# itsakeyfut/renderer-rs

Measured on AMD Instinct MI355X. Metric: Mtris/s at 1920x1080 (input triangles per second, whole frame incl. shading + store), higher is better.
Workload: dtype f32+i32; 1 GPU; c2: BASELINE configs[1]: 10k random triangles, flat shade, 1920x1080; triangles=10000, width=1920, height=1080, target_format=B8G8R8A8_SRGB, parallelism=single, frames_in_flight=4, queue_lanes=4

## Files before the change

renderer-rs_amd/csrc/mirhi_api.hip:

```cpp
#include <hip/hip_runtime.h>

#include <algorithm>
#include <atomic>
#include <chrono>
#include <condition_variable>
#include <cmath>
#include <cstdarg>
#include <cstdio>
#include <cstdlib>
#include <cstring>
#include <mutex>
#include <new>
#include <string>
#include <thread>
#include <vector>

#include <dlfcn.h>
#include <hsa/hsa.h>
#include <hsa/hsa_ext_amd.h>
#include <hsa/amd_hsa_signal.h>
#include <rccl/rccl.h>

#include "../../include/mirhi.h"
#include "mirhi_device.h"
// ... 2108 lines not shown
            j.vb = dd.vb; j.camera = dd.camera; j.object = dd.object; j.stride = dd.stride; j.count = count;
            j.words = words; j.slot_base = slots;
            slots += (count + GEOM_THREADS - 1) / GEOM_THREADS * GEOM_THREADS;
            v.jobs.push_back(j); v.out_off.push_back(v.out_bytes);
            v.out_bytes += vs_attr_offset(count) + (((size_t)count * (words - 1u) * 16 + 255) & ~(size_t)255);
            found = v.jobs.size() - 1;
        }
        dd.vs_words = v.jobs[found].words;
        dd.vs_out = (const void*)(uintptr_t)(v.out_off[found] + 1);
        dd.vs_attr = (const void*)(uintptr_t)(v.out_off[found] + vs_attr_offset(v.jobs[found].count) + 1);
    }
    return v;
}

static mirhi_result grow_scope_buffers(Workspace& w, const std::vector<RecordedPass>& passes, const std::vector<ScopePlan>& scopes, const std::vector<VertexPlan>& vertex) {
    mirhi_result r;
    size_t vs_bytes = 0, carry = 0, ord = 0, flat_tris = 0, pd = 0;
    for (size_t pi = 0; pi < passes.size(); pi++) {
        const RecordedPass& pass = passes[pi];
        vs_bytes = std::max(vs_bytes, vertex[pi].out_bytes);
        if ((pass.carry_in || pass.carry_out) && !pass.depth_t.ptr) carry = std::max(carry, (size_t)pass.color_t.width * pass.color_t.height * 4);
        if (scopes[pi].cls.ordered) ord = std::max(ord, scopes[pi].tris * sizeof(TriRec));
        if (scopes[pi].cls.tri_prog && pass.color_t.format == MIRHI_FORMAT_B8G8R8A8_SRGB) flat_tris = std::max<size_t>(flat_tris, pass.total_tris);
        if (pass.draws.size() > 1) pd = std::max(pd, scopes[pi].tris);
    }
    if ((r = grow(&w.vs_out, &w.vs_out_bytes, vs_bytes ? vs_bytes : 256)) != MIRHI_OK) return r;
    if (carry && (r = grow(&w.carry_depth, &w.carry_depth_bytes, carry)) != MIRHI_OK) return r;
    if (ord && (r = grow(&w.ordered, &w.ordered_bytes, ord)) != MIRHI_OK) return r;
    if (flat_tris && (r = grow(&w.flat_color, &w.flat_color_bytes, flat_tris * 4)) != MIRHI_OK) return r;
    if (pd && (r = grow(&w.prim_draw, &w.prim_draw_bytes, pd * 4)) != MIRHI_OK) return r;
    return MIRHI_OK;
}

static PassParams fill_params(const RecordedPass& pass, const ScopePlan& s, const RasterMode& mode, const Workspace& w, size_t max_tiles, unsigned long long* frag_stats) {
    const RecordedPass::Target& ci = pass.color_t;
    const size_t pool_pages = w.bin_pool_bytes / (BIN_PAGE_RECS * sizeof(BinRec));
    PassParams P;
    memset(&P, 0, sizeof P);
    P.width = ci.width; P.height = ci.height;
    P.tiles_x = s.tiles_x; P.tiles_y = s.tiles_y; P.tile_row_begin = s.r0; P.tile_row_end = s.r1; P.tile_row_step = s.rstep;
    P.num_draws = (uint32_t)pass.draws.size(); P.total_tris = pass.total_tris;
    set_raster_choice(P, s.cls, mode, pass.state, w.ordered, pass.first_tri, pass.total_tris);
    memcpy(P.clear_color, pass.info.clear_color, sizeof P.clear_color);
    {
        auto sat = [](float c) { return c > 0.0f ? (c < 1.0f ? c : 1.0f) : 0.0f; };
        auto enc = [&](float c) { c = sat(c); float e = c <= 0.0031308f ? 12.92f * c : 1.055f * std::pow(c, 1.0f / 2.4f) - 0.055f; return (uint32_t)std::nearbyint(sat(e) * 255.0f); };
        P.clear_packed = enc(P.clear_color[2]) | (enc(P.clear_color[1]) << 8) | (enc(P.clear_color[0]) << 16) |
                         ((uint32_t)std::nearbyint(sat(P.clear_color[3]) * 255.0f) << 24);
    }
    P.color_load = pass.info.color_load_op == MIRHI_LOAD_OP_LOAD ? 1u : 0u;
    P.color_format = ci.format;
    P.color = const_cast<uint8_t*>(ci.ptr);
    if (pass.depth_t.ptr) {
        P.depth = (float*)const_cast<uint8_t*>(pass.depth_t.ptr);
        P.depth_load = pass.info.depth_load_op == MIRHI_LOAD_OP_LOAD ? 1u : 0u;
        P.depth_store = pass.info.depth_store_op == MIRHI_STORE_OP_STORE ? 1u : 0u;
    } else if (pass.carry_in || pass.carry_out) {
        P.depth = w.carry_depth;
    }
    if (pass.carry_in) P.depth_load = 1u;
    if (pass.carry_out) P.depth_store = 1u;
    P.prim_out = (uint32_t*)const_cast<uint8_t*>(pass.prim_t.ptr);
    P.bin_pool = w.bin_pool; P.bin_count = w.counters + CTR_BINS; P.bin_cap = s.bins.bin_cap;
    P.bin_table = w.bin_table; P.pool_next = w.counters + CTR_POOL;
    P.pool_dyn_base = s.bins.fixed_pages; P.pool_dyn_pages = (uint32_t)((pool_pages - s.bins.fixed_pages) / 8);
    P.fixed_recs = s.bins.fixed_per_tile * BIN_PAGE_RECS;
    P.big_recs = w.big_recs; P.big_count = w.big_counts; P.big_count_next = w.big_counts + 1; P.big_cap = s.bins.big_cap;
    P.status = w.status_dev;
    P.frag_stats = frag_stats;
    P.first_prim = pass.first_tri;
    P.prim_draw = pass.draws.size() > 1 ? w.prim_draw : nullptr;
    P.flat_color = (s.cls.tri_prog && ci.format == MIRHI_FORMAT_B8G8R8A8_SRGB) ? w.flat_color : nullptr;
    P.resolve_flat_only = (P.flat_color && !P.depth_load && P.color_format != 2u && !P.prim_out && !(P.depth && P.depth_store)) ? 1u : 0u;
    P.sub_cap = s.bins.sub_cap;
    P.count_stride = s.mode.xcd_bins ? (uint32_t)max_tiles : 0u;
    P.depth_only = pass.depth_only ? 1u : 0u;
    if (P.ibl) {
        P.ibl_irradiance = (const float*)pass.ibl.irradiance; P.ibl_prefiltered = (const float*)pass.ibl.prefiltered; P.ibl_lut = (const float*)pass.ibl.lut;
        P.ibl_irr_size = pass.ibl.irr_size; P.ibl_pre_size = pass.ibl.pre_size; P.ibl_pre_levels = pass.ibl.pre_levels; P.ibl_lut_size = pass.ibl.lut_size;
    }
    if (P.sky) {
        const RecordedPass::SkyDraw& k = pass.sky;
        P.sky_visible = k.visible; P.sky_size = k.size; P.sky_levels = k.levels; P.sky_env = (const float*)k.env;
        memcpy(P.sky_a, k.a, sizeof P.sky_a); memcpy(P.sky_b, k.b, sizeof P.sky_b); memcpy(P.sky_scissor, k.scissor, sizeof P.sky_scissor);
        for (int i = 0; i < 3; i++) P.sky_e0[i] = k.e0[i];
        memcpy(P.sky_pos0, k.pos0, sizeof P.sky_pos0); memcpy(P.sky_posx, k.posx, sizeof P.sky_posx); memcpy(P.sky_posy, k.posy, sizeof P.sky_posy);
        P.sky_depth_bits = k.depth_bits; P.sky_compare = k.compare; P.sky_write = k.write; P.sky_prim = k.prim;
    }
    return P;
}

static mirhi_result build_plan(mirhi_cmd* cmd, bool in_submit) {
    const PlanKnobs knobs = PlanKnobs::read();
    mirhi_device* dev = cmd->dev;
    HIP_TRY(hipSetDevice(dev->ordinal));
    if (cmd->lane >= dev->lanes.size()) cmd->lane = 0;
    hipStream_t stream = dev->lanes[cmd->lane];
    cmd->plan_valid = false;
    { mirhi_result rs = settle_pending(cmd, in_submit); if (rs != MIRHI_OK) return rs; }
    Workspace& w = cmd->ws;
    const size_t n = cmd->passes.size();
    {
        uint64_t tris_now = 0;
        for (auto& pass : cmd->passes) tris_now += pass.total_tris - pass.first_tri;
        if (w.spread && (tris_now > 2 * w.spread_tris || 2 * tris_now < w.spread_tris)) w.spread = false;
    }
    mirhi_result r;
    std::vector<ScopePlan> scopes;
    size_t total_draws = 0, max_tiles = 0;
    for (const RecordedPass& pass : cmd->passes) {
        scopes.push_back(plan_scope(dev, pass, w, knobs));
        total_draws += pass.draws.size();
        max_tiles = std::max(max_tiles, scopes.back().tiles());
    }
    if ((r = rearm_workspace(cmd, scopes, max_tiles, stream, knobs)) != MIRHI_OK) return r;
    std::vector<VertexPlan> vertex;
    size_t jobs_total = 0;
    for (const RecordedPass& pass : cmd->passes) { vertex.push_back(vertex_jobs(pass)); jobs_total += vertex.back().jobs.size(); }
    if ((r = grow_scope_buffers(w, cmd->passes, scopes, vertex)) != MIRHI_OK) return r;
    const size_t params_bytes = n * 2 * sizeof(PassParams);
    w.draws_off = (params_bytes + 255) & ~(size_t)255;
    w.jobs_off = (w.draws_off + total_draws * sizeof(DrawDesc) + 255) & ~(size_t)255;
    const size_t block_bytes = w.jobs_off + jobs_total * sizeof(VsJob);
    if ((r = pblock_reserve(w, block_bytes ? block_bytes : 256)) != MIRHI_OK) return r;
    w.params = reinterpret_cast<PassParams*>(w.pblock);
    DrawDesc* const dev_draws = reinterpret_cast<DrawDesc*>(w.pblock + w.draws_off);
    VsJob* const dev_jobs = reinterpret_cast<VsJob*>(w.pblock + w.jobs_off);
    w.pimage.assign(block_bytes, 0);
    w.draws_count = total_draws;

    size_t draws_done = 0, jobs_done = 0;
    w.wide_eligible = false;
    cmd->plan.clear(); cmd->plan_programs.clear(); cmd->plan_tris = 0;
    for (size_t pi = 0; pi < n; pi++) {
        const ScopePlan& s = scopes[pi];
        VertexPlan& v = vertex[pi];
        const RasterMode mode = raster_mode(s.cls, s.tiles(), s.tris, w.spread, w.wide, knobs);
        w.wide_eligible |= mode.wide_eligible;
        PassParams P = fill_params(cmd->passes[pi], s, mode, w, max_tiles, dev->frag_stats);
        P.draws = dev_draws + draws_done;
        P.vs_jobs = dev_jobs + jobs_done;
        P.num_vs_jobs = (uint32_t)v.jobs.size();
        VsJob* const img_jobs = reinterpret_cast<VsJob*>(w.pimage.data() + w.jobs_off) + jobs_done;
        for (size_t j = 0; j < v.jobs.size(); j++) {
            v.jobs[j].out = w.vs_out + v.out_off[j];
            P.vs_total_slots = v.jobs[j].slot_base + (v.jobs[j].count + GEOM_THREADS - 1) / GEOM_THREADS * GEOM_THREADS;
            img_jobs[j] = v.jobs[j];
        }
        jobs_done += v.jobs.size();
        uint32_t slots = 0;
        for (DrawDesc& dd : v.draws) {
            if (dd.vs_words) { dd.vs_out = w.vs_out + ((size_t)(uintptr_t)dd.vs_out - 1); dd.vs_attr = w.vs_out + ((size_t)(uintptr_t)dd.vs_attr - 1); }
            dd.slot_base = slots; slots += (dd.tri_count + GEOM_THREADS - 1) / GEOM_THREADS * GEOM_THREADS;
        }
        P.total_slots = slots;
        if (!v.draws.empty()) memcpy(w.pimage.data() + w.draws_off + draws_done * sizeof(DrawDesc), v.draws.data(), v.draws.size() * sizeof(DrawDesc));
        draws_done += v.draws.size();
        cmd->plan.push_back(P);
        cmd->plan_programs.push_back(s.cls.programs);
        cmd->plan_tris += s.tris;
        for (uint32_t parity = 0; parity < 2; parity++) {
            PassParams Q = P;
            Q.big_count = w.big_counts + parity;
            Q.big_count_next = w.big_counts + (parity ^ 1u);
            Q.active = w.counters + CTR_ACTIVE + parity * 8u * 32u;
            Q.active_prev = w.counters + CTR_ACTIVE + (parity ^ 1u) * 8u * 32u;
            memcpy(w.pimage.data() + (2 * pi + parity) * sizeof(PassParams), &Q, sizeof Q);
        }
    }
    if ((r = pblock_commit(w, stream)) != MIRHI_OK) return r;
    if (!w.pblock_direct) { cmd->last_stream = stream; cmd->last_native = nullptr; cmd->pending = true; }
    { std::lock_guard<std::mutex> lk(dev->mu); cmd->planned = cmd->passes; }
// ... 1 lines not shown
    cmd->plan_valid = true;
    dev->stats.workspace_bytes = w.bytes();
    return MIRHI_OK;
}

extern "C" int mirhi_debug_raster_choice(const uint32_t in[12], char* name, uint32_t name_len, uint32_t grid_block[4]);
extern "C" int mirhi_debug_scope_plan(const uint32_t* in, uint32_t* out, char* name, uint32_t name_len) {
    static float some_map; static TriRec some_recs;
    const PlanKnobs knobs = PlanKnobs::read();
    DepthState s;
    s.key_set = in[0] != 0u; s.test = in[1]; s.compare = in[2]; s.write = in[3]; s.discard = in[4]; s.blend[0] = in[5];
    float clear_depth; memcpy(&clear_depth, &in[6], 4);
    const uint32_t n = in[14];
    if (n > 4u) return -1;
    DrawDesc draws[4];
    memset(draws, 0, sizeof draws);
    for (uint32_t i = 0; i < n; i++) {
        draws[i].program = in[15 + 3 * i];
        if (in[16 + 3 * i]) { draws[i].shadow_map = &some_map; draws[i].shadow_layers = in[16 + 3 * i] == 2u ? 4u : 0u; }
        draws[i].tex_any_mips = in[17 + 3 * i];
    }
    const ScopeClass c = classify_scope(s, clear_depth, draws, n, in[7] != 0u, knobs, n == 1u && draws[0].program == (uint32_t)MIRHI_PROGRAM_SKYBOX);
    const RasterMode m = raster_mode(c, in[8], in[9], in[10] != 0u, in[11], knobs);
    const BinGeometry g = bin_geometry(in[8], in[9], in[9], m.xcd_bins, in[12], knobs);
    const uint32_t words[28] = {c.key.clear_depth_bits, c.key.pred, c.key.zflip, c.key.zmask, c.key.idflip, c.key.strict, c.key.init_zk, c.key.init_idk,
                                c.ordered, c.masked_plain, c.tri_prog, c.shadowed, c.ibl, c.own_family, c.programs,
                                m.tp_max_area, m.teams, m.wide_eligible, m.xcd_bins, m.wide, m.xcd_swizzle,
                                g.bin_cap, g.sub_cap, g.fixed_per_tile, g.fixed_pages, (uint32_t)g.pages, (uint32_t)((uint64_t)g.pages >> 32), g.big_cap};
    memcpy(out, words, sizeof words);
    PassParams P{};
    set_raster_choice(P, c, m, s, &some_recs, 0u, in[9]);
    const uint32_t choice[12] = {c.programs, in[13], P.pred, P.zflip, P.zmask, P.tp_max_area, P.raster_teams, P.raster_wide, P.alpha_scope, P.xcd_swizzle, P.ordered_recs ? 1u : 0u, 0u};
    return mirhi_debug_raster_choice(choice, name, name_len, out + 28);
}

static mirhi_result stats_params_for(mirhi_cmd* c) {
    Workspace& w = c->ws;
    if (w.stats_params_valid) return MIRHI_OK;
    size_t pixels = 0;
    for (const PassParams& P : c->plan) pixels = std::max(pixels, (size_t)P.width * P.height);
    mirhi_result r;
    if ((r = grow(&w.stats_prim, &w.stats_prim_bytes, (pixels ? pixels : 1) * 4)) != MIRHI_OK) return r;
    if ((r = grow(&w.stats_params, &w.stats_params_bytes, (c->plan.size() ? c->plan.size() : 1) * 2 * sizeof(PassParams))) != MIRHI_OK) return r;
    std::vector<PassParams> copies;
    for (const PassParams& P0 : c->plan)
        for (uint32_t parity = 0; parity < 2; parity++) {
            PassParams P = P0;
            P.big_count = w.big_counts + parity;
            P.big_count_next = w.big_counts + (parity ^ 1u);
            P.active = w.counters + CTR_ACTIVE + parity * 8u * 32u;
            P.active_prev = w.counters + CTR_ACTIVE + (parity ^ 1u) * 8u * 32u;
            P.prim_out = w.stats_prim;
            P.resolve_flat_only = 0u;
            copies.push_back(P);
        }
    if (!copies.empty()) {
        c->dev->foreign_writes++;
        HIP_TRY(hipMemcpyAsync(w.stats_params, copies.data(), copies.size() * sizeof(PassParams), hipMemcpyHostToDevice, c->dev->stream));
        HIP_TRY(hipStreamSynchronize(c->dev->stream));
    }
    w.stats_params_valid = true;
    return MIRHI_OK;
}

static mirhi_result timing_begin(mirhi_device* dev, uint32_t kernel, uint32_t lane, LaunchTiming* t) {
    hipEvent_t ev[2];
// ... 819 lines not shown
```

renderer-rs_amd/csrc/mirhi_device.h:

```cpp
#pragma once
#include <stddef.h>
#include <stdint.h>

namespace mirhi {

constexpr int TILE = 32;
constexpr int TILE_LOG2 = 5;
constexpr int BLOCK = 8;
constexpr int RASTER_THREADS = 256;
constexpr int RASTER_CHUNK = 192;
constexpr int TP_MIN_LANES = 32;
constexpr int GEOM_THREADS = 64;
constexpr int MAX_BIN_SPAN = 4;
constexpr float GUARD_PX = 16000.0f;
constexpr int BIN_PAGE_RECS = 64;
constexpr int BIN_PAGE_LOG2 = 6;
constexpr int BIN_TABLE_ROW = 64;
constexpr int POOL_COUNTER_STRIDE = 32;
constexpr uint32_t BIN_COUNT_STRIDE = 16;
constexpr uint32_t PAGE_EMPTY = 0xFFFFFFFFu;
constexpr uint32_t PAGE_NONE = 0xFFFFFFFEu;
constexpr uint32_t NO_PRIM = 0xFFFFFFFFu;
constexpr uint32_t MAX_PRIM_ID = 0xFFFFFFFDu;

// ... 70 lines not shown
    uint32_t num_draws, total_tris;
    uint32_t total_slots;
    const DrawDesc* draws;
    const VsJob* vs_jobs; uint32_t num_vs_jobs, vs_total_slots;
    uint32_t zflip, zmask, idflip;
    uint32_t strict;
    uint32_t pred;
    uint32_t init_zk, init_idk;
    uint32_t clear_depth_bits;
    float    clear_color[4];
    uint32_t clear_packed;
    uint32_t color_load;
    uint32_t color_format;
    void*    color;
    float*   depth;
    uint32_t depth_load, depth_store;
    uint32_t* prim_out;
    BinRec*   bin_pool; uint32_t* bin_count; uint32_t bin_cap;
    uint32_t* bin_table;
    uint32_t* pool_next;
    uint32_t  pool_dyn_base, pool_dyn_pages;
    uint32_t  fixed_recs;
    BigRec*   big_recs; uint32_t* big_count; uint32_t big_cap;
    uint32_t* big_count_next;
    uint32_t* prim_draw;
    uint32_t  first_prim;
    uint32_t* flat_color;
    uint32_t tp_max_area;
    uint32_t xcd_swizzle;
    uint32_t raster_teams;
    uint32_t sub_cap, count_stride;
    uint32_t raster_wide;
    uint32_t resolve_flat_only;
    uint32_t* active; uint32_t* active_prev;
    TriRec*  ordered_recs; uint32_t ordered_first, ordered_count;
    uint32_t ord_depth_test, ord_depth_write, ord_depth_op;
    uint32_t blend[8];
    uint32_t alpha_scope;
    uint32_t* status;
    unsigned long long* frag_stats;
    uint32_t depth_only;
    uint32_t shadowed;
    uint32_t ibl;
    uint32_t ibl_irr_size, ibl_pre_size, ibl_pre_levels, ibl_lut_size, ibl_pad;
    const float* ibl_irradiance; const float* ibl_prefiltered; const float* ibl_lut;
    uint32_t sky;
    uint32_t sky_visible;
    uint32_t sky_size, sky_levels;
    const float* sky_env;
    int32_t  sky_a[3], sky_b[3];
    int32_t  sky_scissor[4];
    long long sky_e0[3];
    float    sky_pos0[3], sky_posx[3], sky_posy[3];
    uint32_t sky_depth_bits;
    uint32_t sky_compare, sky_write;
    uint32_t sky_prim;
};
static_assert(sizeof(PassParams) % 8 == 0, "PassParams holds pointers");

struct GeometryHead {
    const DrawDesc* draws; uint32_t num_draws;
    uint32_t tris_per_wave;
    const uint8_t* vb0; uint32_t stride0, first0, tris0;
};
struct RasterHead {
    uint32_t* bin_count; const BinRec* bin_pool; uint32_t* big_count;
// ... 12 lines not shown
```

renderer-rs_amd/csrc/mirhi_raster.hip.h:

```cpp
#ifndef MIRHI_RASTER_HIP_H
#define MIRHI_RASTER_HIP_H

#pragma clang fp contract(off)

#ifndef MIRHI_STAGE_PRIO
#define MIRHI_STAGE_PRIO 0
#endif

struct PixelState { uint32_t zk[4], idk[4]; };
struct RecRegs { uint4 w0, w1, w2, w3; };

__device__ __forceinline__ RecRegs load_rec(const uint4* lds_rec, uint32_t j) {
    RecRegs r;
    r.w0 = lds_rec[j * 4u + 0]; r.w1 = lds_rec[j * 4u + 1]; r.w2 = lds_rec[j * 4u + 2]; r.w3 = lds_rec[j * 4u + 3];
    return r;
}

__device__ __forceinline__ int32_t mad24(int32_t a, int32_t b, int32_t c) {
    int32_t d;
    asm("v_mad_i32_i24 %0, %1, %2, %3" : "=v"(d) : "v"(a), "v"(b), "v"(c));
    return d;
}

__device__ __forceinline__ int64_t mul24x24(int32_t a, int32_t b) {
    const uint32_t lo = (uint32_t)__mul24(a, b);
    const int32_t hi = __mulhi(a, b);
    return (int64_t)(((uint64_t)(uint32_t)hi << 32) | lo);
}

struct TileTri { int32_t X[3], Y[3]; uint32_t box, z0, zx, zy, idk, boxed; };
__device__ __forceinline__ uint32_t clamp_box(int32_t bx0, int32_t bx1, int32_t by0, int32_t by1) {
    bx0 = bx0 < 0 ? 0 : (bx0 > TILE ? TILE : bx0); by0 = by0 < 0 ? 0 : (by0 > TILE ? TILE : by0);
    bx1 = bx1 > TILE - 1 ? TILE - 1 : (bx1 < -1 ? -1 : bx1); by1 = by1 > TILE - 1 ? TILE - 1 : (by1 < -1 ? -1 : by1);
    return (uint32_t)bx0 | (((uint32_t)bx1 & 0xFFu) << 8) | ((uint32_t)by0 << 16) | ((uint32_t)by1 << 24);
}

__device__ __forceinline__ bool tile_rec_core(uint4 out[4], const int32_t X[3], const int32_t Y[3], int32_t Ptx, int32_t Pty,
                                              int32_t bx0, int32_t bx1, int32_t by0, int32_t by1, float fox, float foy,
                                              uint32_t z0, uint32_t zx, uint32_t zy, uint32_t idk, uint32_t boxed) {
// ... 321 lines not shown
#pragma unroll 1
        for (int32_t ix = bx0; ix <= bx1; ix++) {
            if ((s0 | s1 | s2) >= 0) {
                const float alpha = pbr_base_alpha(D, c, uvk, px_base + (float)ix, py_base + (float)iy);
                if (!(alpha < cutoff)) {
                    const float dx = (float)ix + dxt;
                    const float z = __builtin_fmaf(dy, zy, __builtin_fmaf(dx, zx, z0));
                    uint32_t zk = __float_as_uint(__builtin_amdgcn_fmed3f(z, 0.0f, 1.0f)) & 0x7FFFFFFFu;
                    if (KEYED == 1) zk = (zk ^ P.zflip) & P.zmask;
                    atomicMin(&lds_key[iy * TILE + ix], ((unsigned long long)zk << 32) | idk);
                }
            }
            s0 += A0; s1 += A1; s2 += A2;
        }
        r0 += B0; r1 += B1; r2 += B2;
    }
}

__device__ __forceinline__ void init_key(ParamsRef P, uint32_t px, uint32_t py, bool valid, uint32_t& zk,
                                         uint32_t& idk, uint32_t& zorig) {
    zk = P.init_zk; idk = P.init_idk; zorig = P.clear_depth_bits;
    if (P.depth_load && P.depth && valid) {
        const uint32_t bits = __float_as_uint(P.depth[(size_t)py * P.width + px]);
        zorig = bits;
        if (P.zmask) {
            const uint32_t t = bits ^ P.zflip;
            if (!P.strict) { zk = t; idk = NO_PRIM; }
            else if (t == 0u) { zk = 0u; idk = 0u; }
            else { zk = t - 1u; idk = NO_PRIM; }
        }
    }
}

template <int KEYED, int TP, int CHUNK, int TEAMS, bool BINS, bool MASKED = false, int WPT = 4>
__device__ __forceinline__ void raster_list(const uint4* __restrict__ list, uint32_t n_total, uint32_t tile, uint32_t fixed_recs, const uint32_t* pages, const uint32_t* seg, uint4* lds_rec, uint32_t* lds_box,
                                            uint32_t* lds_count, uint32_t& flip, uint32_t team, uint32_t nteams, unsigned long long* lds_key, uint32_t tx, uint32_t ty,
                                            uint32_t qmask, int32_t ix0, int32_t iy0, float fix0, float fiy0,
                                            ParamsRef P, PixelState& st, uint32_t qbit0, uint32_t tid,
                                            uint32_t lane) {
    const uint32_t fq = (uint32_t)__builtin_amdgcn_readfirstlane((int)(((tid >> 6) + ((tx + ty) & (uint32_t)(WPT - 1))) & (uint32_t)(WPT - 1)));
    const uint32_t ftid = fq * 64u + lane;
    for (uint32_t base0 = 0; base0 < n_total; base0 += (uint32_t)CHUNK * (TEAMS > 1 ? nteams : 1u)) {
        const uint32_t base = base0 + team * (uint32_t)CHUNK;
        __syncthreads();
        uint32_t* const cnt = lds_count + flip;
        if (tid == 0) lds_count[flip ^ 1u] = 0;
        uint32_t txl = tx, tyl = ty;
        asm volatile("" : "+s"(txl), "+s"(tyl));
        const uint32_t i = base + ftid;
        bool hit = false;
        uint4 rec[4]; uint32_t box = 0;
        const bool wave_stages = fq * 64u < (uint32_t)CHUNK && base + fq * 64u < n_total;
        if (wave_stages) {
        if (MIRHI_STAGE_PRIO) __builtin_amdgcn_s_setprio(MIRHI_STAGE_PRIO);
        if (ftid < (uint32_t)CHUNK && i < n_total) {
            TileTri T;
            if (BINS) {
                uint32_t k = 0, j = i;
                if ((TEAMS > 1 || WPT > 4) && seg) {
#pragma unroll
                    for (uint32_t q = 1; q < 8u; q++) k += i >= seg[q] ? 1u : 0u;
                    j = i - seg[k];
                }
                const uint32_t page = j < fixed_recs ? (tile * fixed_recs + j) >> BIN_PAGE_LOG2 : pages[k * 8u + (j >> BIN_PAGE_LOG2)];
                hit = page < PAGE_NONE;
                if (hit) {
                    const uint32_t ri = (page * (uint32_t)BIN_PAGE_RECS + (j & (BIN_PAGE_RECS - 1u))) * 2u;
                    const uint4 w0 = list[ri], w1 = list[ri + 1u];
                    tile_tri_from_bin(T, w0, w1);
                }
            } else {
                const uint4 w0 = list[(size_t)i * 3u], w1 = list[(size_t)i * 3u + 1u], w2 = list[(size_t)i * 3u + 2u];
                const int32_t tpx0 = (int32_t)txl * TILE, tpy0 = (int32_t)tyl * TILE;
                const int32_t minx = (int32_t)(w2.z & 0x7FFFu), maxx = (int32_t)((w2.z >> 16) & 0x7FFFu);
                const int32_t miny = (int32_t)(w2.w & 0xFFFFu), maxy = (int32_t)(w2.w >> 16);
                hit = !(maxx < tpx0 || minx > tpx0 + TILE - 1 || maxy < tpy0 || miny > tpy0 + TILE - 1);
                if (hit) hit = make_tile_rec(rec, box, w0, w1, w2, (int32_t)txl, (int32_t)tyl);
            }
            if (BINS && hit) hit = make_tile_rec(rec, box, T);
        }
        bool small = false, boxed = false;
        if (hit) {
            const uint32_t bw = ((box >> 8) & 0xFF) - (box & 0xFF) + 1u, bh = (box >> 24) - ((box >> 16) & 0xFF) + 1u;
            small = bw * bh <= P.tp_max_area;
            boxed = (rec[3].w & 0x80000000u) != 0u;
        }
        if (MASKED && P.alpha_scope) {
            uint32_t prim = 0u, mydraw = 0xFFFFFFFFu;
            if (hit) {
                prim = P.idflip ? (MAX_PRIM_ID - rec[3].z) : rec[3].z;
                mydraw = P.num_draws > 1 ? find_draw(P, prim) : 0u;
            }
            uint64_t todo = __ballot(hit);
            while (todo) {
                const uint32_t d = (uint32_t)__builtin_amdgcn_readlane((int)mydraw, __ffsll((long long)todo) - 1);
                const bool mine = hit && mydraw == d;
                DrawRef D = const_draws(P.draws)[__builtin_amdgcn_readfirstlane((int)d)];
                if (draw_needs_alpha_test(D)) {
                    const uint32_t mbw = ((box >> 8) & 0xFF) - (box & 0xFF) + 1u, mbh = (box >> 24) - ((box >> 16) & 0xFF) + 1u;
                    const bool walk = mbw * mbh <= 64u || (rec[3].w & 0x80000000u) != 0u;
                    if (mine && walk) {
                        raster_small_masked<KEYED>(D, prim, rec, box, lds_key, P, txl, tyl);
                        hit = false;
                    }
                    if (mine && !walk) { rec[3].w |= MIRHI_REC_MASKED; small = false; }
                }
                todo &= ~__ballot(mine);
            }
        }
        if (TP) {
            const bool wave_tp = __popcll(__ballot(hit && small)) >= TP_MIN_LANES;
            if (hit && (boxed || (small && wave_tp))) {
                raster_small<KEYED>(rec, box, lds_key, P);
                hit = false;
            }
        }
        const uint64_t ball = __ballot(hit);
        uint32_t wbase = 0;
        if (lane == 0 && ball) wbase = atomicAdd(cnt, (uint32_t)__popcll(ball));
        wbase = __builtin_amdgcn_readfirstlane(wbase);
        if (hit) {
            const uint32_t slot = wbase + (uint32_t)__popcll(ball & ((1ull << lane) - 1ull));
            lds_rec[slot * 4u + 0] = rec[0]; lds_rec[slot * 4u + 1] = rec[1];
            lds_rec[slot * 4u + 2] = rec[2]; lds_rec[slot * 4u + 3] = rec[3];
            if (!TP) lds_box[slot] = box;
        }
        if (MIRHI_STAGE_PRIO) __builtin_amdgcn_s_setprio(0);
        }
        __syncthreads();
        const uint32_t n = *cnt;
        flip ^= 1u;
        if (base0 == 0) { STAMP(5); STAGE_END(2u); }
        if (n) raster_chunk<KEYED, TP, MASKED, 16 / WPT>(lds_rec, lds_box, n, qmask, ix0, iy0, fix0, fiy0, P, st, qbit0, lane, txl, tyl);
    }
}

template <int PROGS, int KEYED, int TP, int TEAMS = 1, bool MASKEDV = false, int WPT = 4, int SHADOWV = 0, bool IBLV = false>
#ifndef MIRHI_PROGS2_WAVES
#define MIRHI_PROGS2_WAVES 5
#endif
__device__ __forceinline__ void raster_body(const PassParams* __restrict__ params, const RasterHead& H) {
    ParamsRef P = *(ParamsPtr)(uintptr_t)params;
    constexpr bool WIDE = WPT > 4;
    static_assert(WPT == 4 || WPT == 8 || WPT == 16, "waves per tile");
    static_assert(!WIDE || (TEAMS == 1 && TP != 0 && PROGS >= 2), "the wide variants exist for one-team mesh scopes with the triangle-parallel path");
    constexpr int NB = 16 / WPT;
    constexpr uint32_t TT = (uint32_t)WPT * 64u;
    constexpr int CHUNK = WIDE ? (int)TT : ((TP && PROGS >= 2) ? RASTER_THREADS : RASTER_CHUNK);
    __shared__ uint4 lds_rec[TEAMS][CHUNK * 4];
    __shared__ unsigned long long lds_key[TP ? TILE * TILE : 1];
    __shared__ uint32_t lds_box[TP ? 1 : RASTER_CHUNK];
    __shared__ uint32_t lds_count[TEAMS * 2];
    const uint32_t tid = threadIdx.x & (TT - 1u), lane = tid & 63u;
    const uint32_t team = TEAMS > 1 ? __builtin_amdgcn_readfirstlane(threadIdx.x >> 8) : 0u;
    const uint32_t q = __builtin_amdgcn_readfirstlane(tid >> 6);
    uint32_t tx = blockIdx.x, tyr = blockIdx.y;
    if (gridDim.y == 1u && P.xcd_swizzle > 1u) {
        const uint32_t G = P.xcd_swizzle, ntiles = gridDim.x;
        uint32_t t = blockIdx.x;
        if (ntiles % (8u * G) == 0u) {
            const uint32_t xcd = blockIdx.x & 7u, j = blockIdx.x >> 3;
            t = ((j / G) * 8u + xcd) * G + (j % G);
        }
        tx = t % H.tiles_x; tyr = t / H.tiles_x;
    }
    const uint32_t tile = tyr * H.tiles_x + tx, ty = H.tile_row_begin + tyr * H.tile_row_step;
    const int32_t ix0 = WPT == 16 ? (int32_t)((q & 3u) * 8u + (lane & 7u)) : (int32_t)((q & 1u) * 16u + (lane & 7u));
    const int32_t iy0 = WPT == 16 ? (int32_t)((q >> 2) * 8u + (lane >> 3)) : (WPT == 8 ? (int32_t)((q >> 1) * 8u + (lane >> 3)) : (int32_t)((q >> 1) * 16u + (lane >> 3)));
    const float fix0 = (float)ix0, fiy0 = (float)iy0;
    const uint32_t qbit0 = WPT == 16 ? (1u << q) : (WPT == 8 ? (1u << ((q >> 1) * 4u + (q & 1u) * 2u)) : (1u << ((q >> 1) * 8u + (q & 1u) * 2u)));
    const uint32_t qmask = WPT == 16 ? qbit0 : (WPT == 8 ? qbit0 * 0x3u : qbit0 * 0x33u);

    STAMP(0);
    __shared__ uint32_t lds_seg[(TEAMS > 1 || WIDE) ? 9 : 1];
    const bool xcd_bins = (TEAMS > 1 || WIDE) && H.count_stride != 0u;
    uint32_t count_raw = H.bin_count[tile * BIN_COUNT_STRIDE];
    const uint32_t nbig_raw = *H.big_count;
    if (TEAMS > 1 || WIDE) {
        if (xcd_bins) {
            if (threadIdx.x == 0) {
                uint32_t c[8];
#pragma unroll
                for (uint32_t k = 0; k < 8u; k++) c[k] = H.bin_count[(k * H.count_stride + tile) * BIN_COUNT_STRIDE];
                uint32_t acc = 0;
#pragma unroll
// ... 42 lines not shown
                    if (P.prim_out) P.prim_out[pix] = NO_PRIM;
                }
                if (write_depth) P.depth[pix] = __uint_as_float(P.clear_depth_bits);
            }
        }
        STAMP(4);
        return;
    }

    if (tid == 0) { lds_count[2u * team] = 0; lds_count[2u * team + 1u] = 0; }
    if (PROGS >= 2 && tid == 0 && team == 0) __hip_atomic_fetch_add(&P.active[(tile & 7u) * 32u], 1u, __ATOMIC_RELAXED, __HIP_MEMORY_SCOPE_AGENT);
    uint32_t flip = 0;
    if (TP) for (uint32_t e = tid + team * TT; e < TILE * TILE; e += TT * nteams) lds_key[e] = ~0ull;
    PixelState st;
#pragma unroll
    for (int b = 0; b < 4; b++) { st.zk[b] = P.init_zk; st.idk[b] = P.init_idk; }
    if (TEAMS > 1 && team != 0u) {
#pragma unroll
        for (int b = 0; b < 4; b++) { st.zk[b] = KEYED == 0 ? 0x7FFFFFFFu : 0xFFFFFFFFu; st.idk[b] = 0xFFFFFFFFu; }
    }
    if (P.depth_load && P.depth && team == 0) {
        const uint32_t px0 = tx * TILE + (uint32_t)ix0, py0 = ty * TILE + (uint32_t)iy0;
#pragma unroll
        for (int b = 0; b < NB; b++) {
            const uint32_t px = px0 + (uint32_t)(b & 1) * BLOCK, py = py0 + (uint32_t)(b >> 1) * BLOCK;
            uint32_t zo;
            init_key(P, px, py, px < P.width && py < P.height, st.zk[b], st.idk[b], zo);
        }
    }

    STAMP(1);
    STAGE_END(1u);
    constexpr bool MASKED = MASKEDV && PROGS == 4 && TP != 0;
    if (count) raster_list<KEYED, TP, CHUNK, TEAMS, true, MASKED, WPT>(reinterpret_cast<const uint4*>(H.bin_pool), count, tile, H.fixed_recs, lds_pages, xcd_bins ? lds_seg : nullptr, lds_rec[team], lds_box, lds_count + 2u * team, flip, team, nteams, lds_key, tx, ty, qmask, ix0, iy0, fix0, fiy0, P, st,
                                                         qbit0, tid, lane);
    STAMP(2);
    if (count && tid == 0 && team == 0) {
        H.bin_count[tile * BIN_COUNT_STRIDE] = 0;
        if (xcd_bins) for (uint32_t k = 1; k < 8u; k++) H.bin_count[(k * H.count_stride + tile) * BIN_COUNT_STRIDE] = 0;
    }
    if (need_pages && threadIdx.x < (uint32_t)BIN_TABLE_ROW) launder_params((ParamsPtr)(uintptr_t)params)->bin_table[tile * (uint32_t)BIN_TABLE_ROW + threadIdx.x] = PAGE_EMPTY;
    if (nbig) raster_list<KEYED, TP, CHUNK, TEAMS, false, MASKED, WPT>(reinterpret_cast<const uint4*>(launder_params((ParamsPtr)(uintptr_t)params)->big_recs), nbig, tile, 0u, lds_pages, nullptr, lds_rec[team], lds_box, lds_count + 2u * team, flip, team, nteams, lds_key, tx, ty, qmask, ix0, iy0, fix0, fiy0, P, st,
                                                         qbit0, tid, lane);

    STAMP(3);
    STAGE_END(3u);
    if (TP || TEAMS > 1) __syncthreads();
    if (TP) {
#pragma unroll
        for (int b = 0; b < NB; b++) {
            const unsigned long long kreg = ((unsigned long long)st.zk[b] << 32) | st.idk[b];
            const unsigned long long klds = lds_key[(iy0 + (b >> 1) * BLOCK) * TILE + ix0 + (b & 1) * BLOCK];
            const unsigned long long kmin = klds < kreg ? klds : kreg;
            st.zk[b] = (uint32_t)(kmin >> 32); st.idk[b] = (uint32_t)kmin;
        }
    }
    if (TEAMS > 1 && !solo) {
        unsigned long long* const mine = reinterpret_cast<unsigned long long*>(&lds_rec[team][0]);
        if (team != 0u) {
#pragma unroll
            for (int b = 0; b < 4; b++) mine[b * RASTER_THREADS + tid] = ((unsigned long long)st.zk[b] << 32) | st.idk[b];
        }
        __syncthreads();
        if (team == 0u) {
#pragma unroll
            for (int b = 0; b < 4; b++) {
                unsigned long long k = ((unsigned long long)st.zk[b] << 32) | st.idk[b];
#pragma unroll
                for (int t = 1; t < TEAMS; t++) {
                    const unsigned long long o = reinterpret_cast<const unsigned long long*>(&lds_rec[t][0])[b * RASTER_THREADS + tid];
                    k = o < k ? o : k;
                }
                mine[b * RASTER_THREADS + tid] = k;
                st.zk[b] = (uint32_t)(k >> 32); st.idk[b] = (uint32_t)k;
            }
        }
// ... 8 lines not shown
    }
    if constexpr (PROGS == 0) {
        if (!(P.depth && P.depth_store)) return;
        const uint32_t px0 = tx * TILE + (uint32_t)ix0, py0 = ty * TILE + (uint32_t)iy0;
        uint32_t held = 0;
        bool held_all = false;
#pragma unroll
        for (int b = 0; b < NB; b++) {
            const uint32_t px = px0 + (uint32_t)(b & 1) * BLOCK, py = py0 + (uint32_t)(b >> 1) * BLOCK;
            const bool inb = px < P.width && py < P.height;
            uint32_t izk, iidk, zorig;
            init_key(P, px, py, inb, izk, iidk, zorig);
            const uint32_t zkb = st.zk[b], idb = st.idk[b];
            const bool none = !inb || ((zkb == izk) && (idb == iidk));
            const uint32_t zb = (none || !P.zmask) ? zorig : (zkb ^ P.zflip);
            uint32_t* const dimg = reinterpret_cast<uint32_t*>(P.depth);
            const bool all = __ballot(inb) == ~0ull;
            if (NB < 2) { if (inb) dimg[(size_t)py * P.width + px] = zb; continue; }
            if ((b & 1) == 0) { held = zb; held_all = all; if (!all && inb) dimg[(size_t)py * P.width + px] = zb; }
            else if (all && held_all) store_pair(dimg, py * P.width + (px - (uint32_t)BLOCK) - (lane & 7u), held, zb, lane);
            else {
                if (held_all) dimg[(size_t)py * P.width + px - BLOCK] = held;
                if (inb) dimg[(size_t)py * P.width + px] = zb;
            }
        }
        STAMP(4);
        return;
    }
    const ParamsPtr R = launder_params((ParamsPtr)(uintptr_t)params);
    const uint32_t px0 = tx * TILE + (uint32_t)ix0, py0 = ty * TILE + (uint32_t)iy0;
    uint32_t flat4[4] = {0u, 0u, 0u, 0u};
    const uint8_t* flat_color = PROGS == 1 && !R->depth_load ? reinterpret_cast<const uint8_t*>(R->flat_color) : nullptr;
    const uint32_t init_idk = R->init_idk;
    if (flat_color) {
        if (R->idflip) {
#pragma unroll
            for (int b = 0; b < 4; b++)
                if (st.idk[b] != init_idk) flat4[b] = *reinterpret_cast<const uint32_t*>(flat_color + ((MAX_PRIM_ID - st.idk[b]) << 2));
        } else {
#pragma unroll
            for (int b = 0; b < 4; b++)
                if (st.idk[b] != init_idk) flat4[b] = *reinterpret_cast<const uint32_t*>(flat_color + (st.idk[b] << 2));
        }
    }
    if (PROGS == 1 && R->resolve_flat_only) {
        const bool need_shade = (st.idk[0] != init_idk && flat4[0] == 0u) || (st.idk[1] != init_idk && flat4[1] == 0u) ||
                                (st.idk[2] != init_idk && flat4[2] == 0u) || (st.idk[3] != init_idk && flat4[3] == 0u);
        if (__ballot(need_shade) == 0ull) {
            const uint32_t width = R->width, height = R->height, clear_packed = R->clear_packed;
            uint8_t* row0 = reinterpret_cast<uint8_t*>(R->color);
            uint8_t* row1 = row0 + (size_t)BLOCK * width * 4u;
            const uint32_t off = (py0 * width + px0) * 4u;
            if ((tx + 1u) * TILE <= width && (ty + 1u) * TILE <= height && !R->color_load) {
                store_target(reinterpret_cast<uint32_t*>(row0 + off), st.idk[0] != init_idk ? flat4[0] : clear_packed);
                store_target(reinterpret_cast<uint32_t*>(row0 + off + 4u * BLOCK), st.idk[1] != init_idk ? flat4[1] : clear_packed);
                store_target(reinterpret_cast<uint32_t*>(row1 + off), st.idk[2] != init_idk ? flat4[2] : clear_packed);
                store_target(reinterpret_cast<uint32_t*>(row1 + off + 4u * BLOCK), st.idk[3] != init_idk ? flat4[3] : clear_packed);
            } else {
                const uint32_t color_load = R->color_load;
#pragma unroll
                for (int b = 0; b < 4; b++) {
                    const uint32_t px = px0 + (uint32_t)(b & 1) * BLOCK, py = py0 + (uint32_t)(b >> 1) * BLOCK;
                    const bool won = st.idk[b] != init_idk;
                    if (px < width && py < height && (won || !color_load))
                        store_target(reinterpret_cast<uint32_t*>((b >> 1 ? row1 : row0) + off + 4u * BLOCK * (uint32_t)(b & 1)), won ? flat4[b] : clear_packed);
                }
            }
            STAMP(4);
            return;
        }
    }
    uint32_t held = 0;
    bool held_all = false;
#pragma unroll 1
    for (int b = 0; b < NB; b++) {
        if (TEAMS > 1 && !solo && (uint32_t)(b * TEAMS) / 4u != team) continue;
        const uint32_t px = px0 + (uint32_t)(b & 1) * BLOCK, py = py0 + (uint32_t)(b >> 1) * BLOCK;
        const bool inb = px < P.width && py < P.height;
        uint32_t izk, iidk, zorig;
        init_key(P, px, py, inb, izk, iidk, zorig);
        const uint32_t zkb = b == 0 ? st.zk[0] : (b == 1 ? st.zk[1] : (b == 2 ? st.zk[2] : st.zk[3]));
        const uint32_t idb = b == 0 ? st.idk[0] : (b == 1 ? st.idk[1] : (b == 2 ? st.idk[2] : st.idk[3]));
        const bool none = !inb || ((zkb == izk) && (idb == iidk));
        const size_t pix = (size_t)py * P.width + px;
        const uint32_t prim = none ? NO_PRIM : (P.idflip ? (MAX_PRIM_ID - idb) : idb);
        f4 col = {P.clear_color[0], P.clear_color[1], P.clear_color[2], P.clear_color[3]};
        const uint32_t mydraw = none ? 0xFFFFFFFFu : (P.num_draws > 1 ? find_draw(P, prim) : 0u);
        uint32_t flat = 0;
        if (PROGS == 1 && P.flat_color && !none) {
            if (P.depth_load) flat = P.flat_color[prim];
            else flat = b == 0 ? flat4[0] : (b == 1 ? flat4[1] : (b == 2 ? flat4[2] : flat4[3]));
        }
        uint64_t todo = __ballot(!none && flat == 0u);
        while (todo) {
            const uint32_t d = (uint32_t)__builtin_amdgcn_readlane((int)mydraw, __ffsll((long long)todo) - 1);
            const bool mine = mydraw == d && flat == 0u;
            if (mine) {
                DrawRef D = const_draws(P.draws)[__builtin_amdgcn_readfirstlane(mydraw)];
                const uint32_t tri = prim - D.prim_base;
                const float pxc = (float)px + 0.5f, pyc = (float)py + 0.5f;
                if constexpr (IBLV) col = (D.program == 0) ? shade_triangle_program(D, tri, pxc, pyc)
                                                            : shade_model_program<true, SHADOWV, true>(D, tri, pxc, pyc, SHADOWV == 2 ? __uint_as_float(zkb ^ P.zflip) : 0.0f, R);
// ... 67 lines not shown
```

renderer-rs_amd/csrc/mirhi_scope.h:

```cpp
#pragma once
#include <algorithm>
#include <cstdlib>
#include <cstring>
#include <unistd.h>

#include "../../include/mirhi.h"
#include "mirhi_device.h"
#include "mirhi_variant.h"

namespace mirhi {

struct DepthState {
    bool key_set = false;
    uint32_t test = 0, compare = 0, write = 0, discard = 0;
    uint32_t blend[8] = {0, 0, 0, 0, 0, 0, 0, 0};
    bool operator==(const DepthState& o) const {
        return key_set == o.key_set && test == o.test && compare == o.compare && write == o.write && discard == o.discard && memcmp(blend, o.blend, sizeof blend) == 0;
    }
    bool order_dependent_depth() const { return test && write && compare == MIRHI_COMPARE_NOT_EQUAL; }
};

inline bool ordering_compare(uint32_t op) {
    return op == MIRHI_COMPARE_LESS || op == MIRHI_COMPARE_LESS_OR_EQUAL || op == MIRHI_COMPARE_GREATER || op == MIRHI_COMPARE_GREATER_OR_EQUAL;
}
// ... 24 lines not shown
        static const uint32_t bits[8] = {0u, 1u, 2u, 3u, 4u, 5u, 6u, 7u};
        P.pred = bits[op & 7u] | (op == MIRHI_COMPARE_ALWAYS ? 8u : 0u);
        if (P.pred == 0) P.pred = 16u;
        P.zflip = 0; P.zmask = 0xFFFFFFFFu; P.idflip = 1; P.strict = 0;
        P.init_zk = cbits; P.init_idk = NO_PRIM;
        return P;
    }
    const bool greater = (op == MIRHI_COMPARE_GREATER || op == MIRHI_COMPARE_GREATER_OR_EQUAL);
    P.strict = (op == MIRHI_COMPARE_LESS || op == MIRHI_COMPARE_GREATER) ? 1u : 0u;
    P.zflip = greater ? 0xFFFFFFFFu : 0u;
    P.zmask = 0xFFFFFFFFu;
    P.idflip = P.strict ? 0u : 1u;
    const uint32_t t = cbits ^ P.zflip;
    if (!P.strict) { P.init_zk = t; P.init_idk = NO_PRIM; }
    else if (t == 0u) { P.init_zk = 0u; P.init_idk = 0u; }
    else { P.init_zk = t - 1u; P.init_idk = NO_PRIM; }
    return P;
}

struct PlanKnobs {
    struct Knob { bool set = false; int value = 0; };
    Knob masked_ordered;
    Knob tp_density;
    Knob tp_max_area;
    Knob raster_teams;
    Knob xcd_bins;
    Knob raster_wide;
    Knob bin_cap;
    Knob fixed_pages;
    Knob pool_pages;
    Knob always_clear;
    Knob xcd_run;
    Knob verify_idle;
    static PlanKnobs read() {
        static const struct { const char* name; Knob PlanKnobs::*field; } table[] = {
            {"MASKED_ORDERED", &PlanKnobs::masked_ordered}, {"TP_DENSITY", &PlanKnobs::tp_density}, {"TP_MAX_AREA", &PlanKnobs::tp_max_area},
            {"RASTER_TEAMS", &PlanKnobs::raster_teams}, {"XCD_BINS", &PlanKnobs::xcd_bins}, {"RASTER_WIDE", &PlanKnobs::raster_wide},
            {"BIN_CAP", &PlanKnobs::bin_cap}, {"FIXED_PAGES", &PlanKnobs::fixed_pages}, {"POOL_PAGES", &PlanKnobs::pool_pages},
            {"ALWAYS_CLEAR", &PlanKnobs::always_clear}, {"XCD_RUN", &PlanKnobs::xcd_run}, {"VERIFY_IDLE", &PlanKnobs::verify_idle}};
        PlanKnobs k;
        for (char** e = environ; e && *e; e++) {
            if (strncmp(*e, "MIRHI_", 6) != 0) continue;
            const char* name = *e + 6;
            const char* eq = strchr(name, '=');
            if (!eq) continue;
            for (const auto& t : table) {
                Knob& knob = k.*t.field;
                if (!knob.set && strlen(t.name) == (size_t)(eq - name) && strncmp(name, t.name, (size_t)(eq - name)) == 0) { knob.set = true; knob.value = atoi(eq + 1); }
            }
        }
        return k;
    }
};

struct ScopeClass {
    DepthKey key;
    bool ordered;
    bool masked_plain;
    bool tri_prog;
    bool has_draws;
    uint32_t shadowed;
    uint32_t ibl;
    bool own_family;
    uint32_t programs;
    bool sky;
};

inline ScopeClass classify_scope(const DepthState& s, float clear_depth, const DrawDesc* draws, size_t n, bool depth_only, const PlanKnobs& knobs, bool sky = false) {
    ScopeClass c{};
    c.key = depth_key_setup(s, clear_depth);
    if (sky) {
        c.sky = true; c.has_draws = true; c.own_family = true; c.programs = PROGS_SKY;
        return c;
    }
    c.masked_plain = s.key_set && s.discard && s.blend[0] == 0 && !s.order_dependent_depth() && !(knobs.masked_ordered.set && knobs.masked_ordered.value != 0) &&
                     c.key.pred == 0u;
    c.ordered = s.key_set && (s.blend[0] != 0 || (s.discard != 0 && !c.masked_plain) || s.order_dependent_depth());
    c.has_draws = n != 0;
    uint32_t progs = 0;
    for (size_t i = 0; i < n; i++) {
        const DrawDesc& dd = draws[i];
        c.tri_prog |= dd.program == MIRHI_PROGRAM_TRIANGLE;
        c.shadowed |= dd.shadow_map ? (dd.shadow_layers ? 2u : 1u) : 0u;
        c.ibl |= dd.program == MIRHI_PROGRAM_MODEL_PBR_IBL ? 1u : 0u;
        progs |= dd.program == MIRHI_PROGRAM_TRIANGLE ? PROGS_TRIANGLE : ((dd.program == MIRHI_PROGRAM_MODEL_PBR || dd.program == MIRHI_PROGRAM_MODEL_PBR_IBL || dd.tex_any_mips || dd.tex_srgb) ? PROGS_PBR : PROGS_MODEL);
    }
// ... 73 lines not shown
```

Before: 1157 Mtris/s.

## Carry flat colour with raster records in LDS instead of per-pixel global lookup

When a tile's triangle list fits in one chunk, each binned triangle's flat colour is fetched at record-build time and stored in an LDS side table. The record's id key is shifted left by eight bits so its low byte holds the LDS slot. The resolve stage then reads pixel colours from LDS instead of doing gather loads from the global flat_color array per pixel, and restores the original ids afterwards. This costs one extra global load per binned triangle and a small LDS array, and limits the prim-id range that can be keyed.

```diff
diff --git a/renderer-rs_amd/csrc/mirhi_api.hip b/renderer-rs_amd/csrc/mirhi_api.hip
--- a/renderer-rs_amd/csrc/mirhi_api.hip
+++ b/renderer-rs_amd/csrc/mirhi_api.hip
@@ -2164,7 +2164,7 @@
     return MIRHI_OK;
 }
 
-static PassParams fill_params(const RecordedPass& pass, const ScopePlan& s, const RasterMode& mode, const Workspace& w, size_t max_tiles, unsigned long long* frag_stats) {
+static PassParams fill_params(const RecordedPass& pass, const ScopePlan& s, const RasterMode& mode, const Workspace& w, size_t max_tiles, unsigned long long* frag_stats, const PlanKnobs& knobs) {
     const RecordedPass::Target& ci = pass.color_t;
     const size_t pool_pages = w.bin_pool_bytes / (BIN_PAGE_RECS * sizeof(BinRec));
     PassParams P;
@@ -2204,6 +2204,8 @@
     P.prim_draw = pass.draws.size() > 1 ? w.prim_draw : nullptr;
     P.flat_color = (s.cls.tri_prog && ci.format == MIRHI_FORMAT_B8G8R8A8_SRGB) ? w.flat_color : nullptr;
     P.resolve_flat_only = (P.flat_color && !P.depth_load && P.color_format != 2u && !P.prim_out && !(P.depth && P.depth_store)) ? 1u : 0u;
+    P.rec_colour = rec_colour_scope(P.total_tris, P.flat_color != nullptr, P.depth_load != 0u, knobs) ? 1u : 0u;
+    P.rec_bias = rec_colour_bias(P.idflip);
     P.sub_cap = s.bins.sub_cap;
     P.count_stride = s.mode.xcd_bins ? (uint32_t)max_tiles : 0u;
     P.depth_only = pass.depth_only ? 1u : 0u;
@@ -2269,7 +2271,7 @@
         VertexPlan& v = vertex[pi];
         const RasterMode mode = raster_mode(s.cls, s.tiles(), s.tris, w.spread, w.wide, knobs);
         w.wide_eligible |= mode.wide_eligible;
-        PassParams P = fill_params(cmd->passes[pi], s, mode, w, max_tiles, dev->frag_stats);
+        PassParams P = fill_params(cmd->passes[pi], s, mode, w, max_tiles, dev->frag_stats, knobs);
         P.draws = dev_draws + draws_done;
         P.vs_jobs = dev_jobs + jobs_done;
         P.num_vs_jobs = (uint32_t)v.jobs.size();
@@ -2337,6 +2339,12 @@
     set_raster_choice(P, c, m, s, &some_recs, 0u, in[9]);
     const uint32_t choice[12] = {c.programs, in[13], P.pred, P.zflip, P.zmask, P.tp_max_area, P.raster_teams, P.raster_wide, P.alpha_scope, P.xcd_swizzle, P.ordered_recs ? 1u : 0u, 0u};
     return mirhi_debug_raster_choice(choice, name, name_len, out + 28);
+}
+
+extern "C" void mirhi_debug_rec_colour(const uint32_t in[4], uint32_t out[2]) {
+    const PlanKnobs knobs = PlanKnobs::read();
+    out[0] = rec_colour_scope(in[0], in[3] != 0u, in[2] != 0u, knobs) ? 1u : 0u;
+    out[1] = rec_colour_bias(in[1]);
 }
 
 static mirhi_result stats_params_for(mirhi_cmd* c) {
diff --git a/renderer-rs_amd/csrc/mirhi_device.h b/renderer-rs_amd/csrc/mirhi_device.h
--- a/renderer-rs_amd/csrc/mirhi_device.h
+++ b/renderer-rs_amd/csrc/mirhi_device.h
@@ -126,6 +126,8 @@
     uint32_t sub_cap, count_stride;
     uint32_t raster_wide;
     uint32_t resolve_flat_only;
+    uint32_t rec_colour;
+    uint32_t rec_bias;
     uint32_t* active; uint32_t* active_prev;
     TriRec*  ordered_recs; uint32_t ordered_first, ordered_count;
     uint32_t ord_depth_test, ord_depth_write, ord_depth_op;
diff --git a/renderer-rs_amd/csrc/mirhi_raster.hip.h b/renderer-rs_amd/csrc/mirhi_raster.hip.h
--- a/renderer-rs_amd/csrc/mirhi_raster.hip.h
+++ b/renderer-rs_amd/csrc/mirhi_raster.hip.h
@@ -5,6 +5,9 @@
 
 #ifndef MIRHI_STAGE_PRIO
 #define MIRHI_STAGE_PRIO 0
+#endif
+#ifndef MIRHI_RASTER_REC_COLOUR
+#define MIRHI_RASTER_REC_COLOUR 1
 #endif
 
 struct PixelState { uint32_t zk[4], idk[4]; };
@@ -392,12 +395,12 @@
     }
 }
 
-template <int KEYED, int TP, int CHUNK, int TEAMS, bool BINS, bool MASKED = false, int WPT = 4>
+template <int KEYED, int TP, int CHUNK, int TEAMS, bool BINS, bool MASKED = false, int WPT = 4, bool RECCOL = false>
 __device__ __forceinline__ void raster_list(const uint4* __restrict__ list, uint32_t n_total, uint32_t tile, uint32_t fixed_recs, const uint32_t* pages, const uint32_t* seg, uint4* lds_rec, uint32_t* lds_box,
                                             uint32_t* lds_count, uint32_t& flip, uint32_t team, uint32_t nteams, unsigned long long* lds_key, uint32_t tx, uint32_t ty,
                                             uint32_t qmask, int32_t ix0, int32_t iy0, float fix0, float fiy0,
                                             ParamsRef P, PixelState& st, uint32_t qbit0, uint32_t tid,
-                                            uint32_t lane) {
+                                            uint32_t lane, uint32_t* lds_col = nullptr, bool rc = false, uint32_t colbase = 0u) {
     const uint32_t fq = (uint32_t)__builtin_amdgcn_readfirstlane((int)(((tid >> 6) + ((tx + ty) & (uint32_t)(WPT - 1))) & (uint32_t)(WPT - 1)));
     const uint32_t ftid = fq * 64u + lane;
     for (uint32_t base0 = 0; base0 < n_total; base0 += (uint32_t)CHUNK * (TEAMS > 1 ? nteams : 1u)) {
@@ -410,6 +413,7 @@
         const uint32_t i = base + ftid;
         bool hit = false;
         uint4 rec[4]; uint32_t box = 0;
+        uint32_t reccol = 0u;
         const bool wave_stages = fq * 64u < (uint32_t)CHUNK && base + fq * 64u < n_total;
         if (wave_stages) {
         if (MIRHI_STAGE_PRIO) __builtin_amdgcn_s_setprio(MIRHI_STAGE_PRIO);
@@ -427,6 +431,7 @@
                 if (hit) {
                     const uint32_t ri = (page * (uint32_t)BIN_PAGE_RECS + (j & (BIN_PAGE_RECS - 1u))) * 2u;
                     const uint4 w0 = list[ri], w1 = list[ri + 1u];
+                    if constexpr (RECCOL) { if (rc) reccol = P.flat_color[P.idflip ? (MAX_PRIM_ID - w1.w) : w1.w]; }
                     tile_tri_from_bin(T, w0, w1);
                 }
             } else {
@@ -435,6 +440,7 @@
                 const int32_t minx = (int32_t)(w2.z & 0x7FFFu), maxx = (int32_t)((w2.z >> 16) & 0x7FFFu);
                 const int32_t miny = (int32_t)(w2.w & 0xFFFFu), maxy = (int32_t)(w2.w >> 16);
                 hit = !(maxx < tpx0 || minx > tpx0 + TILE - 1 || maxy < tpy0 || miny > tpy0 + TILE - 1);
+                if constexpr (RECCOL) { if (rc && hit) reccol = P.flat_color[P.idflip ? (MAX_PRIM_ID - w2.y) : w2.y]; }
                 if (hit) hit = make_tile_rec(rec, box, w0, w1, w2, (int32_t)txl, (int32_t)tyl);
             }
             if (BINS && hit) hit = make_tile_rec(rec, box, T);
@@ -481,6 +487,12 @@
         wbase = __builtin_amdgcn_readfirstlane(wbase);
         if (hit) {
             const uint32_t slot = wbase + (uint32_t)__popcll(ball & ((1ull << lane) - 1ull));
+            if constexpr (RECCOL) {
+                if (rc) {
+                    rec[3].z = ((rec[3].z - P.rec_bias) << 8) | (colbase + slot);
+                    lds_col[colbase + slot] = reccol;
+                }
+            }
             lds_rec[slot * 4u + 0] = rec[0]; lds_rec[slot * 4u + 1] = rec[1];
             lds_rec[slot * 4u + 2] = rec[2]; lds_rec[slot * 4u + 3] = rec[3];
             if (!TP) lds_box[slot] = box;
@@ -511,6 +523,8 @@
     __shared__ unsigned long long lds_key[TP ? TILE * TILE : 1];
     __shared__ uint32_t lds_box[TP ? 1 : RASTER_CHUNK];
     __shared__ uint32_t lds_count[TEAMS * 2];
+    constexpr bool RECCOL = MIRHI_RASTER_REC_COLOUR != 0 && PROGS == 1 && TP == 0 && TEAMS == 1 && WPT == 4 && KEYED != 2 && !MASKEDV && CHUNK <= 256;
+    __shared__ uint32_t lds_col[RECCOL ? CHUNK : 1];
     const uint32_t tid = threadIdx.x & (TT - 1u), lane = tid & 63u;
     const uint32_t team = TEAMS > 1 ? __builtin_amdgcn_readfirstlane(threadIdx.x >> 8) : 0u;
     const uint32_t q = __builtin_amdgcn_readfirstlane(tid >> 6);
@@ -619,16 +633,17 @@
     STAMP(1);
     STAGE_END(1u);
     constexpr bool MASKED = MASKEDV && PROGS == 4 && TP != 0;
-    if (count) raster_list<KEYED, TP, CHUNK, TEAMS, true, MASKED, WPT>(reinterpret_cast<const uint4*>(H.bin_pool), count, tile, H.fixed_recs, lds_pages, xcd_bins ? lds_seg : nullptr, lds_rec[team], lds_box, lds_count + 2u * team, flip, team, nteams, lds_key, tx, ty, qmask, ix0, iy0, fix0, fiy0, P, st,
-                                                         qbit0, tid, lane);
+    const bool rc = RECCOL && P.rec_colour != 0u && count + nbig <= (uint32_t)CHUNK;
+    if (count) raster_list<KEYED, TP, CHUNK, TEAMS, true, MASKED, WPT, RECCOL>(reinterpret_cast<const uint4*>(H.bin_pool), count, tile, H.fixed_recs, lds_pages, xcd_bins ? lds_seg : nullptr, lds_rec[team], lds_box, lds_count + 2u * team, flip, team, nteams, lds_key, tx, ty, qmask, ix0, iy0, fix0, fiy0, P, st,
+                                                         qbit0, tid, lane, lds_col, rc, 0u);
     STAMP(2);
     if (count && tid == 0 && team == 0) {
         H.bin_count[tile * BIN_COUNT_STRIDE] = 0;
         if (xcd_bins) for (uint32_t k = 1; k < 8u; k++) H.bin_count[(k * H.count_stride + tile) * BIN_COUNT_STRIDE] = 0;
     }
     if (need_pages && threadIdx.x < (uint32_t)BIN_TABLE_ROW) launder_params((ParamsPtr)(uintptr_t)params)->bin_table[tile * (uint32_t)BIN_TABLE_ROW + threadIdx.x] = PAGE_EMPTY;
-    if (nbig) raster_list<KEYED, TP, CHUNK, TEAMS, false, MASKED, WPT>(reinterpret_cast<const uint4*>(launder_params((ParamsPtr)(uintptr_t)params)->big_recs), nbig, tile, 0u, lds_pages, nullptr, lds_rec[team], lds_box, lds_count + 2u * team, flip, team, nteams, lds_key, tx, ty, qmask, ix0, iy0, fix0, fiy0, P, st,
-                                                         qbit0, tid, lane);
+    if (nbig) raster_list<KEYED, TP, CHUNK, TEAMS, false, MASKED, WPT, RECCOL>(reinterpret_cast<const uint4*>(launder_params((ParamsPtr)(uintptr_t)params)->big_recs), nbig, tile, 0u, lds_pages, nullptr, lds_rec[team], lds_box, lds_count + 2u * team, flip, team, nteams, lds_key, tx, ty, qmask, ix0, iy0, fix0, fiy0, P, st,
+                                                         qbit0, tid, lane, lds_col, rc, count);
 
     STAMP(3);
     STAGE_END(3u);
@@ -703,7 +718,16 @@
     uint32_t flat4[4] = {0u, 0u, 0u, 0u};
     const uint8_t* flat_color = PROGS == 1 && !R->depth_load ? reinterpret_cast<const uint8_t*>(R->flat_color) : nullptr;
     const uint32_t init_idk = R->init_idk;
-    if (flat_color) {
+    bool from_rec = false;
+    if constexpr (RECCOL) {
+        if (rc) {
+            from_rec = true;
+#pragma unroll
+            for (int b = 0; b < 4; b++)
+                if (st.idk[b] != init_idk) flat4[b] = lds_col[st.idk[b] & 0xFFu];
+        }
+    }
+    if (!from_rec && flat_color) {
         if (R->idflip) {
 #pragma unroll
             for (int b = 0; b < 4; b++)
@@ -739,6 +763,14 @@
             }
             STAMP(4);
             return;
+        }
+    }
+    if constexpr (RECCOL) {
+        if (rc) {
+            const uint32_t bias = R->rec_bias;
+#pragma unroll
+            for (int b = 0; b < 4; b++)
+                if (st.idk[b] != init_idk) st.idk[b] = (st.idk[b] >> 8) + bias;
         }
     }
     uint32_t held = 0;
diff --git a/renderer-rs_amd/csrc/mirhi_scope.h b/renderer-rs_amd/csrc/mirhi_scope.h
--- a/renderer-rs_amd/csrc/mirhi_scope.h
+++ b/renderer-rs_amd/csrc/mirhi_scope.h
@@ -80,12 +80,14 @@
     Knob always_clear;
     Knob xcd_run;
     Knob verify_idle;
+    Knob rec_colour;
     static PlanKnobs read() {
         static const struct { const char* name; Knob PlanKnobs::*field; } table[] = {
             {"MASKED_ORDERED", &PlanKnobs::masked_ordered}, {"TP_DENSITY", &PlanKnobs::tp_density}, {"TP_MAX_AREA", &PlanKnobs::tp_max_area},
             {"RASTER_TEAMS", &PlanKnobs::raster_teams}, {"XCD_BINS", &PlanKnobs::xcd_bins}, {"RASTER_WIDE", &PlanKnobs::raster_wide},
             {"BIN_CAP", &PlanKnobs::bin_cap}, {"FIXED_PAGES", &PlanKnobs::fixed_pages}, {"POOL_PAGES", &PlanKnobs::pool_pages},
-            {"ALWAYS_CLEAR", &PlanKnobs::always_clear}, {"XCD_RUN", &PlanKnobs::xcd_run}, {"VERIFY_IDLE", &PlanKnobs::verify_idle}};
+            {"ALWAYS_CLEAR", &PlanKnobs::always_clear}, {"XCD_RUN", &PlanKnobs::xcd_run}, {"VERIFY_IDLE", &PlanKnobs::verify_idle},
+            {"REC_COLOUR", &PlanKnobs::rec_colour}};
         PlanKnobs k;
         for (char** e = environ; e && *e; e++) {
             if (strncmp(*e, "MIRHI_", 6) != 0) continue;
@@ -100,6 +102,13 @@
         return k;
     }
 };
+
+constexpr uint32_t REC_COLOUR_KEY_MAX = 0xFFFFFEu;
+inline uint32_t rec_colour_bias(uint32_t idflip) { return idflip ? MAX_PRIM_ID - REC_COLOUR_KEY_MAX : 0u; }
+inline bool rec_colour_scope(uint32_t total_tris, bool flat_colours, bool depth_load, const PlanKnobs& knobs) {
+    if (knobs.rec_colour.set && knobs.rec_colour.value == 0) return false;
+    return flat_colours && !depth_load && total_tris <= REC_COLOUR_KEY_MAX + 1u;
+}
 
 struct ScopeClass {
     DepthKey key;
```

After: 1165 Mtris/s (median of 6 runs). Within noise of the previous version (+0.6%).
